# eliasandronicou/split-learning-k8s

Measured on AMD Instinct MI355X. Metric: training samples/sec (node) for split CNN, higher is better.
Workload: dtype fp32; 1 GPU; K2: split CNN (model_def.py ModelPartA+ModelPartB) both stages fused on 1xMI355X, synthetic 1x28x28 MNIST-shape batches, fp32, HIP-graph step; global_batch=4096, per_gpu_batch=4096, topology=fused-1gpu, graph=True, conv=x3, cut_handoff=client conv1 writes the x3 split input images (slk_conv1_fwd_x3); no f32 cut, client_backward=fused into the x3 dgrad (slk_conv2_dgrad_x3_c1w); no cut gradient in HBM

## Files before the change

### split-learning-k8s_amd/csrc/slk_x3.hip

```cpp
#include "slk_common.h"

#include <type_traits>

using namespace slk;

typedef _Float16 f16x8 __attribute__((ext_vector_type(8)));
typedef _Float16 f16x2 __attribute__((ext_vector_type(2)));

namespace {

constexpr int X3_SMAX = 126;
__device__ __forceinline__ int x3_exp(float amax) {
    if (!(amax > 0.f) || !__builtin_isfinite(amax)) return 0;
    int e;
    (void)frexpf(amax, &e);
    return min(14 - e, X3_SMAX);
}
__device__ __forceinline__ float x3_unscale(float v, float u1, float u2) { return (v * u1) * u2; }

__device__ __forceinline__ void x3_split8(const float* v, float sc, f16x8& h, f16x8& l) {
#pragma unroll
    for (int k = 0; k < 8; k += 2) {
        const float a = v[k] * sc, b = v[k + 1] * sc;
        const _Float16 ha = (_Float16)a, hb = (_Float16)b;
// ... 922 lines not shown
            }
        } else {
            float* gb = cut_grad + (size_t)b * A_SAMPLE + (16 * nt + n16) * A_PIX;
#pragma unroll
            for (int i = 0; i < X3D_MPW; ++i) {
                const int t = T0 + g + 4 * i, p = 16 * t + 4 * kc;
                if (t < T1 && p < A_PIX)
                    *reinterpret_cast<float4*>(gb + p) =
                        make_float4(x3_unscale(acc[i][0], us1, us2), x3_unscale(acc[i][1], us1, us2),
                                    x3_unscale(acc[i][2], us1, us2), x3_unscale(acc[i][3], us1, us2));
            }
        }
        ++q;
    }
    X3D_TS(127, 7);
    if constexpr (C1W) {
        __syncthreads();
        const float* part = reinterpret_cast<const float*>(d1s);
        if (tid < C1 * 10) {
            const int ci = tid / 10, j = tid - (tid / 10) * 10;
            const int ntc = ci >> 4, cl = ci & 15;
            const int src = ((cl >> 2) * 16 + j) * 4 + (cl & 3);
            float sum = 0.f;
            for (int gg = 0; gg < 4; ++gg) sum += part[(ntc + 2 * gg) * 256 + src];
            c1slabs[(size_t)blockIdx.x * (C1 * 10) + (j < 9 ? ci * 9 + j : C1 * 9 + ci)] = sum * ldexpf(1.f, -sw);
        }
    }
}

constexpr int X3W_THREADS = 512;
constexpr int X3W_Q = 192;
constexpr int X3W_DYP = X3W_Q * 64;
constexpr int X3W_XP = 260 * 64;
constexpr int X3W_BUF = 2 * X3W_DYP + 2 * X3W_XP;
constexpr int X3W_NKS = 128;
constexpr int X3W_XITEMS = 260 * 4;
constexpr int X3W_XR = (X3W_XITEMS + X3W_THREADS - 1) / X3W_THREADS;
constexpr int X3W_DYITEMS = 48 * 8;
static_assert(X3W_DYITEMS % 64 == 0, "whole waves of dY items");
static_assert(2 * X3W_BUF <= 163840, "LDS");

__global__ __launch_bounds__(X3W_THREADS, 1) void conv2_wgrad_x3_kernel(
    const float* __restrict__ act, const float* __restrict__ act_amax, const float* __restrict__ dpooled,
    const float* __restrict__ dp_amax, const uint8_t* __restrict__ code, float* __restrict__ slabs, int B) {
    __shared__ __attribute__((aligned(1024))) char smem[2 * X3W_BUF];
    const int tid = threadIdx.x, lane = tid & 63;
    const int wave = __builtin_amdgcn_readfirstlane(tid >> 6);
    const int h = wave & 1, kp = (wave >> 1) & 1, tg = wave >> 2;
    const int nks = (int)gridDim.x / 2;
    const int bid = blockIdx.x;
    const bool xcd = (nks & 7) == 0;
    const int cohalf = xcd ? (bid >> 3) & 1 : bid & 1;
    const int ks = xcd ? (bid >> 4) * 8 + (bid & 7) : bid >> 1;
    const int U = 3 * B;
    float* red = reinterpret_cast<float*>(smem);

    float ma = 0.f, md = 0.f;
    for (int i = tid; i < B; i += X3W_THREADS) {
        ma = fmaxf(ma, act_amax[i]);
        md = fmaxf(md, dp_amax[i]);
    }
    ma = wave_max(ma);
    md = wave_max(md);
    if (lane == 0) {
        red[wave] = ma;
        red[8 + wave] = md;
    }
    __syncthreads();
    ma = red[0];
    md = red[8];
#pragma unroll
    for (int i = 1; i < 8; ++i) {
        ma = fmaxf(ma, red[i]);
        md = fmaxf(md, red[8 + i]);
    }
    __syncthreads();
    const int sx = x3_exp(ma), sd = x3_exp(md);
    int sb_ld = 0;

    float xv[X3W_XR][8];
    auto load_x = [&](int uu) {
        const int b = uu / 3, t3 = uu - (uu / 3) * 3;
        const float* base = act + (size_t)b * A_SAMPLE + t3 * 8 * A_HW;
#pragma unroll
        for (int r = 0; r < X3W_XR; ++r) {
            const int i = min(tid + r * X3W_THREADS, X3W_XITEMS - 1);
            const int cg = i & 3, p = i >> 2;
#pragma unroll
            for (int j = 0; j < 8; ++j) xv[r][j] = base[(8 * cg + j) * A_PIX + p];
        }
    };
    auto split_x = [&](char* img) {
        const float xsc = ldexpf(1.f, sb_ld);
#pragma unroll
        for (int r = 0; r < X3W_XR; ++r) {
            const int i = min(tid + r * X3W_THREADS, X3W_XITEMS - 1);
            const int cg = i & 3, p = i >> 2;
            f16x8 hh, ll;
            x3_split8(xv[r], xsc, hh, ll);
            char* o = img + 2 * X3W_DYP + p * 64 + cg * 16;
            *reinterpret_cast<f16x8*>(o) = hh;
            *reinterpret_cast<f16x8*>(o + X3W_XP) = ll;
        }
    };
    const int ditem = min(tid, X3W_DYITEMS - 1);
    const int dg = ditem & 7, dw = ditem >> 3;
    float dv[4];
    uint32_t dcb[4];
    auto load_dy = [&](int uu) {
        const int b = uu / 3, t3 = uu - (uu / 3) * 3;
        const int w = (4 * t3 + dw / 12) * P_HW + dw % 12;
        const size_t o = (size_t)b * P_SAMPLE + (32 * cohalf + 4 * dg) * P_WIN + w;
#pragma unroll
        for (int j = 0; j < 4; ++j) {
            dv[j] = dpooled[o + j * P_WIN];
            dcb[j] = code[o + j * P_WIN];
        }
        sb_ld = max(x3_exp(act_amax[b]), sx);
    };
    float dbacc[4] = {0.f, 0.f, 0.f, 0.f};
    auto store_dy = [&](char* img, bool real) {
        const float dsc = ldexpf(1.f, sd + sx - sb_ld);
        const bool mine = real && tid < X3W_DYITEMS;
#pragma unroll
        for (int j = 0; j < 4; ++j) dbacc[j] = (mine && dcb[j] != (uint32_t)CODE_NONE) ? dbacc[j] + dv[j] : dbacc[j];
        uint32_t hv[2], lv[2];
#pragma unroll
        for (int j = 0; j < 4; j += 2) {
            const float a = dv[j] * dsc, c = dv[j + 1] * dsc;
            const _Float16 ha = (_Float16)a, hc = (_Float16)c;
            const _Float16 la = (_Float16)(a - (float)ha), lc = (_Float16)(c - (float)hc);
            hv[j / 2] = __builtin_bit_cast(uint32_t, f16x2{ha, hc});
            lv[j / 2] = __builtin_bit_cast(uint32_t, f16x2{la, lc});
        }
        const uint32_t dc = dcb[0] | (dcb[1] << 8) | (dcb[2] << 16) | (dcb[3] << 24);
        const uint32_t cA = __builtin_amdgcn_perm(0u, dc, 0x01010000u), cB = __builtin_amdgcn_perm(0u, dc, 0x03030202u);
        const int wy = dw / 12, wx = dw % 12;
        const int pf = dw & 1;
#pragma unroll
        for (int pos0 = 0; pos0 < 4; ++pos0) {
            const int pos = pos0 ^ pf;
            const uint32_t T = 0xFFu << (8 * pos);
            const uint32_t mA = __builtin_amdgcn_perm(0u, T, cA), mB = __builtin_amdgcn_perm(0u, T, cB);
            const int q = (2 * wy + (pos >> 1)) * 24 + 2 * wx + (pos & 1);
            char* o = img + q * 64 + ((((dg >> 2) ^ (q >> 3)) & 1) * 32) + 8 * (dg & 3);
            *reinterpret_cast<uint2*>(o) = make_uint2(hv[0] & mA, hv[1] & mB);
            *reinterpret_cast<uint2*>(o + X3W_DYP) = make_uint2(lv[0] & mA, lv[1] & mB);
        }
    };

    const int g4 = lane >> 4, qq = (lane >> 2) & 3, pp = lane & 3;
    int abase[3][2];
    int xbase[3][3];
#pragma unroll
    for (int j = 0; j < 3; ++j) {
        const int idx = 2 * (kp + 2 * j) + (g4 >> 1);
        const int orow = 2 * (idx / 3) + (g4 & 1), seg = idx % 3;
        const int q0 = 24 * orow + 8 * seg;
#pragma unroll
        for (int mi = 0; mi < 2; ++mi) abase[j][mi] = (q0 + qq) * 64 + ((mi ^ ((q0 >> 3) & 1)) * 32) + pp * 8;
#pragma unroll
        for (int kx = 0; kx < 3; ++kx) {
            const int x = 8 * seg + qq + kx;
            xbase[j][kx] = 2 * X3W_DYP + ((orow * A_HW + x) * 64) + h * 32 + pp * 8;
        }
    }
    typedef __fp16 hf4 __attribute__((__vector_size__(8)));
    typedef _Float16 f16x4 __attribute__((ext_vector_type(4)));
    typedef __attribute__((address_space(3))) hf4* lp4;
    auto trr = [&](const char* p) -> f16x8 {
        const f16x4 lo = __builtin_bit_cast(f16x4, __builtin_amdgcn_ds_read_tr16_b64_v4f16((lp4)p));
        const f16x4 hi = __builtin_bit_cast(f16x4, __builtin_amdgcn_ds_read_tr16_b64_v4f16((lp4)(p + 4 * 64)));
        return __builtin_shufflevector(lo, hi, 0, 1, 2, 3, 4, 5, 6, 7);
    };

    f32x4 acc[2][5];
#pragma unroll
    for (int mi = 0; mi < 2; ++mi)
#pragma unroll
        for (int t = 0; t < 5; ++t) acc[mi][t] = f32x4{0.f, 0.f, 0.f, 0.f};

    auto unit_mfma = [&](const char* img, auto TG) {
        constexpr int T0 = decltype(TG)::value ? 5 : 0, NT = decltype(TG)::value ? 4 : 5;
        constexpr int N = 3 * NT;
        f16x8 Ah[2][2], Al[2][2], Bh[3], Bl[3];
        auto rdA = [&](int j, int slot) {
#pragma unroll
            for (int mi = 0; mi < 2; ++mi) {
                Ah[slot][mi] = trr(img + abase[j][mi]);
                Al[slot][mi] = trr(img + X3W_DYP + abase[j][mi]);
            }
        };
        auto rdB = [&](int n, int slot) {
            const int j = n / NT, tap = T0 + n % NT;
            const int to = (tap / 3) * A_HW * 64;
            Bh[slot] = trr(img + xbase[j][tap % 3] + to);
            Bl[slot] = trr(img + X3W_XP + xbase[j][tap % 3] + to);
        };
        rdA(0, 0);
        rdB(0, 0);
        rdB(1, 1);
#pragma unroll
        for (int n = 0; n < N; ++n) {
            if (n + 2 < N) {
                rdB(n + 2, (n + 2) % 3);
                if ((n + 2) % NT == 0) rdA((n + 2) / NT, ((n + 2) / NT) & 1);
            }
            const int j = n / NT, t = n % NT;
#pragma unroll
            for (int mi = 0; mi < 2; ++mi)
                acc[mi][t] = mfma_x3(Ah[j & 1][mi], Al[j & 1][mi], Bh[n % 3], Bl[n % 3], acc[mi][t]);
        }
        __builtin_amdgcn_sched_group_barrier(0x100, 16, 0);
#pragma unroll
        for (int n = 0; n < N; ++n) {
            __builtin_amdgcn_sched_group_barrier(0x008, 6, 0);
            if (n + 2 < N) {
                if ((n + 2) % NT == 0) __builtin_amdgcn_sched_group_barrier(0x100, 12, 0);
                else __builtin_amdgcn_sched_group_barrier(0x100, 4, 0);
            }
        }
    };

    const int per = (U + nks - 1) / nks;
    const int u0 = min(ks * per, U), u1 = min(u0 + per, U);
    int u = u0;
    if (u < u1) {
        load_x(u);
        load_dy(u);
        split_x(smem);
        store_dy(smem, true);
        load_x(min(u + 1, u1 - 1));
        load_dy(min(u + 1, u1 - 1));
    }
    int k = 0;
#pragma unroll 1
    for (; u < u1; ++u, ++k) {
        __syncthreads();
        const int nx = u + 1, nx2 = u + 2;
        const char* img = smem + (k & 1) * X3W_BUF;
        char* nimg = smem + ((k & 1) ^ 1) * X3W_BUF;
        store_dy(nimg, nx < u1);
        split_x(nimg);
        load_x(min(nx2, u1 - 1));
        load_dy(min(nx2, u1 - 1));
        if (tg == 0) unit_mfma(img, std::integral_constant<int, 0>{});
        else unit_mfma(img, std::integral_constant<int, 1>{});
    }
    asm volatile("s_waitcnt vmcnt(0)" ::: "memory");
    __syncthreads();
    constexpr int XN = 2 * 5 * 4;
    float* xch = reinterpret_cast<float*>(smem) + (h + 2 * tg) * (XN * 64);
    if (kp == 1) {
#pragma unroll
        for (int mi = 0; mi < 2; ++mi) {
#pragma unroll
            for (int t = 0; t < 5; ++t)
#pragma unroll
                for (int r = 0; r < 4; ++r) xch[((mi * 5 + t) * 4 + r) * 64 + lane] = acc[mi][t][r];
        }
    }
    float* dbs = reinterpret_cast<float*>(smem) + 4 * XN * 64;
    if (tid < X3W_DYITEMS)
#pragma unroll
        for (int j = 0; j < 4; ++j) dbs[tid * 4 + j] = dbacc[j];
    __syncthreads();
    if (tid < 32) {
        const int g = tid >> 2, j = tid & 3;
        float sum = 0.f;
        for (int w = 0; w < 48; ++w) sum += dbs[(w * 8 + g) * 4 + j];
        slabs[(size_t)ks * (W2_N + C2) + W2_N + 32 * cohalf + tid] = sum;
    }
    if (kp == 0) {
        const float us1 = ldexpf(1.f, -sx), us2 = ldexpf(1.f, -sd);
        float* slab = slabs + (size_t)ks * (W2_N + C2);
        const int ci = 16 * h + (lane & 15);
        const int nt = tg ? 4 : 5;
#pragma unroll
        for (int mi = 0; mi < 2; ++mi) {
#pragma unroll
            for (int t = 0; t < 5; ++t)
                if (t < nt)
#pragma unroll
                    for (int r = 0; r < 4; ++r) {
                        const int co = 32 * cohalf + 16 * mi + 4 * (lane >> 4) + r;
                        slab[(co * C1 + ci) * 9 + 5 * tg + t] =
                            x3_unscale(acc[mi][t][r] + xch[((mi * 5 + t) * 4 + r) * 64 + lane], us1, us2);
                    }
        }
    }
}

constexpr int X3P_THREADS = 512;
constexpr int X3P_STEPS = 3;
constexpr int X3P_REC = X3P_STEPS * 4 * 64 * 16;
constexpr int X3P_IDXB = X3P_STEPS * 4 * 64 * 2;
constexpr int X3P_DYOFF = 2 * X3F_PLANE;
constexpr int X3P_IDXOFF = X3P_DYOFF + 2 * X3P_REC;
constexpr int X3P_BUF = (X3P_IDXOFF + X3P_IDXB + 1023) / 1024 * 1024;
constexpr int X3P_ITEMS = C2 * 12;
constexpr int X3P_SBN = (163840 - 2 * X3P_BUF) / 4;
static_assert(2 * X3P_BUF <= 163840 && X3P_ITEMS <= 2 * X3P_THREADS && X3P_ITEMS > X3P_THREADS, "x3p layout");

template <int TGI>
struct X3pTaps {
    static constexpr int NT = TGI == 0 ? 3 : 2;
    static constexpr int tap(int t) { return TGI == 0 ? t : (TGI == 1 ? 3 + t : (TGI == 2 ? 5 + t : 7 + t)); }
};

template <int TGI>
__device__ __forceinline__ void x3p_steps(const char* img, const int (&pb)[X3P_STEPS][4], const int (&sw)[3], int arec,
                                          int aidx, f32x4 (&acc)[3][4]) {
    using TT = X3pTaps<TGI>;
    constexpr int NT = TT::NT;
    typedef __fp16 hf4 __attribute__((__vector_size__(8)));
    typedef _Float16 f16x4 __attribute__((ext_vector_type(4)));
    typedef _Float16 f16x16 __attribute__((ext_vector_type(16)));
    typedef __attribute__((address_space(3))) hf4* lp4;
    auto tr = [&](const char* p) -> f16x4 { return __builtin_bit_cast(f16x4, __builtin_amdgcn_ds_read_tr16_b64_v4f16((lp4)p)); };
#pragma unroll
    for (int s = 0; s < X3P_STEPS; ++s) {
        f16x8 ah[4], al[4];
        int ix[4];
#pragma unroll
        for (int mt = 0; mt < 4; ++mt) {
            ah[mt] = *reinterpret_cast<const f16x8*>(img + X3P_DYOFF + arec + s * 4096 + mt * 256);
            al[mt] = *reinterpret_cast<const f16x8*>(img + X3P_DYOFF + X3P_REC + arec + s * 4096 + mt * 256);
            ix[mt] = *reinterpret_cast<const uint16_t*>(img + X3P_IDXOFF + aidx + s * 512 + mt * 32);
        }
#pragma unroll
        for (int t = 0; t < NT; ++t) {
            const int tap = TT::tap(t), ky = tap / 3, kx = tap % 3;
            f16x4 bh[4], bl[4];
#pragma unroll
            for (int jb = 0; jb < 4; ++jb) {
                const char* p = img + pb[s][jb] + sw[kx] + (ky * A_HW + kx) * 64;
                bh[jb] = tr(p);
                bl[jb] = tr(p + X3F_PLANE);
            }
            const f16x16 Bh = __builtin_shufflevector(__builtin_shufflevector(bh[0], bh[1], 0, 1, 2, 3, 4, 5, 6, 7),
                                                      __builtin_shufflevector(bh[2], bh[3], 0, 1, 2, 3, 4, 5, 6, 7),
                                                      0, 1, 2, 3, 4, 5, 6, 7, 8, 9, 10, 11, 12, 13, 14, 15);
            const f16x16 Bl = __builtin_shufflevector(__builtin_shufflevector(bl[0], bl[1], 0, 1, 2, 3, 4, 5, 6, 7),
                                                      __builtin_shufflevector(bl[2], bl[3], 0, 1, 2, 3, 4, 5, 6, 7),
                                                      0, 1, 2, 3, 4, 5, 6, 7, 8, 9, 10, 11, 12, 13, 14, 15);
#pragma unroll
            for (int mt = 0; mt < 4; ++mt) {
                f32x4 c = acc[t][mt];
                c = __builtin_amdgcn_smfmac_f32_16x16x64_f16(ah[mt], Bh, c, ix[mt], 0, 0);
                c = __builtin_amdgcn_smfmac_f32_16x16x64_f16(ah[mt], Bl, c, ix[mt], 0, 0);
                c = __builtin_amdgcn_smfmac_f32_16x16x64_f16(al[mt], Bh, c, ix[mt], 0, 0);
                acc[t][mt] = c;
            }
        }
    }
}

__global__ __launch_bounds__(X3P_THREADS, 1) void conv2_wgrad_x3p_kernel(
    const uint16_t* __restrict__ act16, const float* __restrict__ act_amax, const float* __restrict__ dpooled,
    const float* __restrict__ dp_amax, const uint8_t* __restrict__ code, float* __restrict__ slabs, int B) {
    __shared__ __attribute__((aligned(1024))) char smem[163840];
    int* sbt = reinterpret_cast<int*>(smem + 2 * X3P_BUF);
    const int tid = threadIdx.x, lane = tid & 63;
    const int wave = __builtin_amdgcn_readfirstlane(tid >> 6);
    const int h = wave & 1, tgi = ((wave >> 1) & 1) * 2 + (wave >> 2);
    const int ks = blockIdx.x, nks = gridDim.x;
    const int U = 3 * B;
    float* red = reinterpret_cast<float*>(smem);
    X3P_TS(0, 7);

    float ma = 0.f, md = 0.f;
    for (int i = tid; i < B; i += X3P_THREADS) {
        ma = fmaxf(ma, act_amax[i]);
        md = fmaxf(md, dp_amax[i]);
    }
    ma = wave_max(ma);
    md = wave_max(md);
    if (lane == 0) {
        red[wave] = ma;
        red[16 + wave] = md;
    }
    __syncthreads();
    ma = red[0];
    md = red[16];
#pragma unroll
    for (int i = 1; i < 8; ++i) {
        ma = fmaxf(ma, red[i]);
        md = fmaxf(md, red[16 + i]);
    }
    __syncthreads();
    const int sx = x3_exp(ma), sd = x3_exp(md);

    constexpr int NI = 2;
    const int nit = wave < 4 ? 2 : 1;
    int goff[NI], ldo[NI][2];
#pragma unroll
    for (int r = 0; r < NI; ++r) {
        const int q = r == 0 ? wave : 8 + (wave & 3);
        const int wyl = q / 3, wq = q - (q / 3) * 3;
        goff[r] = lane * P_WIN + wyl * P_HW + 4 * wq;
#pragma unroll
        for (int d = 0; d < 2; ++d) {
            const int L = 6 * (2 * wyl + d) + 2 * wq;
            const int st = L >> 4, gb = (L >> 2) & 3, jb = L & 3;
            const int rec = (st * 4 + 2 * (jb >> 1) + (gb >> 1)) * 64 + lane;
            ldo[r][d] = rec * 16 + 8 * (gb & 1);
        }
    }
    float4 dv[NI];
    uint32_t dcw[NI];
    int ld_b = 0, sb0 = 0;
    auto load_dy = [&](int uu) {
        const int b = uu / 3, t3 = uu - (uu / 3) * 3;
        const size_t o = (size_t)b * P_SAMPLE + t3 * 4 * P_HW;
#pragma unroll
        for (int r = 0; r < NI; ++r) {
            if (r < nit) {
                dv[r] = *reinterpret_cast<const float4*>(dpooled + o + goff[r]);
                dcw[r] = *reinterpret_cast<const uint32_t*>(code + o + goff[r]);
            }
        }
        ld_b = b;
    };
    float dbacc[NI] = {};
    int trk = 0;
    (void)trk;
    auto store_dy1 = [&](char* img, bool real, int r) {
        const float dsc = ldexpf(1.f, sbt[ld_b - sb0]);
        {
            {
                const float v[4] = {dv[r].x, dv[r].y, dv[r].z, dv[r].w};
#if SLK_X3D_TRACE
                if (r == 0) {
                    asm volatile("" ::"v"(v[0]), "v"(dcw[0]));
                    X3P_TS(trk, 4);
                }
#endif
                const uint32_t cw = dcw[r];
                const uint32_t ib = (cw & 1u) | ((cw >> 6) & 4u) | ((cw >> 12) & 16u) | ((cw >> 18) & 64u) | 0x88u;
#pragma unroll
                for (int j = 0; j < 4; ++j) {
                    const uint32_t c = (cw >> (8 * j)) & 0xFFu;
                    if (real && c < (uint32_t)CODE_NONE) dbacc[r] += v[j];
                }
                const uint32_t rowp = (cw >> 1) & 0x7F7F7F7Fu;
                uint32_t H[2], Lw[2];
#pragma unroll
                for (int jp = 0; jp < 2; ++jp) {
                    const float a = v[2 * jp] * dsc, bb = v[2 * jp + 1] * dsc;
                    const _Float16 ha = (_Float16)a, hb = (_Float16)bb;
                    const _Float16 la = (_Float16)(a - (float)ha), lb = (_Float16)(bb - (float)hb);
                    H[jp] = __builtin_bit_cast(uint32_t, f16x2{ha, hb});
                    Lw[jp] = __builtin_bit_cast(uint32_t, f16x2{la, lb});
                }
#pragma unroll
                for (int d = 0; d < 2; ++d) {
                    const uint32_t z = (d ? (rowp & ~(rowp >> 1)) : ~(rowp | (rowp >> 1))) & 0x01010101u;
                    const uint32_t m8 = z * 0xFFu;
                    const uint32_t mA = __builtin_amdgcn_perm(0u, m8, 0x01010000u), mB = __builtin_amdgcn_perm(0u, m8, 0x03030202u);
                    char* ph = img + X3P_DYOFF + ldo[r][d];
                    *reinterpret_cast<uint2*>(ph) = make_uint2(H[0] & mA, H[1] & mB);
                    *reinterpret_cast<uint2*>(ph + X3P_REC) = make_uint2(Lw[0] & mA, Lw[1] & mB);
                    img[X3P_IDXOFF + ((ldo[r][d] >> 4) << 1) + ((ldo[r][d] >> 3) & 1)] = (char)ib;
                }
            }
        }
    };
    auto store_dy = [&](char* img, bool real) {
#pragma unroll
        for (int r = 0; r < NI; ++r)
            if (r < nit) store_dy1(img, real, r);
        X3P_TS(trk, 5);
    };

    const int gbl = lane >> 4, qq = (lane >> 2) & 3, pp = lane & 3;
    int pb[X3P_STEPS][4], sw[3];
#pragma unroll
    for (int s = 0; s < X3P_STEPS; ++s)
#pragma unroll
        for (int jb = 0; jb < 4; ++jb) {
            const int L = 16 * s + 4 * gbl + jb, y = L / 6, xb = L - (L / 6) * 6;
            pb[s][jb] = (y * A_HW + 4 * xb + qq) * 64 + pp * 8;
        }
#pragma unroll
    for (int kx = 0; kx < 3; ++kx) sw[kx] = (h ^ (((kx + qq) >> 1) & 1)) * 32;
    const int arec = ((lane >> 4) * 64 + (lane & 15)) * 16, aidx = ((lane >> 4) * 64 + (lane & 15)) * 2;

    f32x4 acc[3][4];
#pragma unroll
    for (int t = 0; t < 3; ++t)
#pragma unroll
        for (int mt = 0; mt < 4; ++mt) acc[t][mt] = f32x4{0.f, 0.f, 0.f, 0.f};

    const int per = (U + nks - 1) / nks;
    const int u0 = min(ks * per, U), u1 = min(u0 + per, U);
    sb0 = u0 / 3;
    const int nsb = u1 > u0 ? (u1 - 1) / 3 - sb0 + 1 : 0;
    for (int j = tid; j < nsb; j += X3P_THREADS) sbt[j] = sd + sx - max(x3_exp(act_amax[sb0 + j]), sx);
    __syncthreads();
    int u = u0;
    if (u < u1) {
        x3_issue_unit_img(act16, u, wave, lane, lds_u32(smem));
        load_dy(u);
        store_dy(smem, true);
        load_dy(min(u + 1, u1 - 1));
    }
    int k = 0;
#pragma unroll 1
    for (; u < u1; ++u, ++k) {
        X3P_TS(k, 6);
        if (nit == 2) asm volatile("s_waitcnt vmcnt(4)" ::: "memory");
        else asm volatile("s_waitcnt vmcnt(2)" ::: "memory");
        __syncthreads();
        X3P_TS(k, 0);
        trk = k;
        const int nx = u + 1, nx2 = u + 2;
        const char* img = smem + (k & 1) * X3P_BUF;
        char* nimg = smem + ((k & 1) ^ 1) * X3P_BUF;
        const bool dfirst = wave >= 4;
        if (dfirst) store_dy(nimg, nx < u1);
        x3_issue_unit_img(act16, min(nx, u1 - 1), wave, lane, lds_u32(nimg));
        if (dfirst) load_dy(min(nx2, u1 - 1));
        X3P_TS(k, 1);
        if (tgi == 0) x3p_steps<0>(img, pb, sw, arec, aidx, acc);
        else if (tgi == 1) x3p_steps<1>(img, pb, sw, arec, aidx, acc);
        else if (tgi == 2) x3p_steps<2>(img, pb, sw, arec, aidx, acc);
        else x3p_steps<3>(img, pb, sw, arec, aidx, acc);
        X3P_TS(k, 2);
        if (!dfirst) {
            store_dy(nimg, nx < u1);
            load_dy(min(nx2, u1 - 1));
        }
        X3P_TS(k, 3);
    }
    X3P_TS(127, 7);
    asm volatile("s_waitcnt vmcnt(0)" ::: "memory");
    __syncthreads();
    float* dbs = reinterpret_cast<float*>(smem);
#pragma unroll
    for (int r = 0; r < NI; ++r)
        if (r < nit) dbs[(r == 0 ? wave : 8 + (wave & 3)) * 64 + lane] = dbacc[r];
    __syncthreads();
    float* slab = slabs + (size_t)ks * (W2_N + C2);
    if (tid < C2) {
        float sum = 0.f;
        for (int q = 0; q < 12; ++q) sum += dbs[q * 64 + tid];
        slab[W2_N + tid] = sum;
    }
    const float us1 = ldexpf(1.f, -sx), us2 = ldexpf(1.f, -sd);
    const int ci = 16 * h + (lane & 15);
    auto write_slab = [&](auto TG) {
        using TT = X3pTaps<decltype(TG)::value>;
#pragma unroll
        for (int t = 0; t < TT::NT; ++t)
#pragma unroll
            for (int mt = 0; mt < 4; ++mt)
#pragma unroll
                for (int r = 0; r < 4; ++r) {
                    const int co = 16 * mt + 4 * (lane >> 4) + r;
                    slab[(co * C1 + ci) * 9 + TT::tap(t)] = x3_unscale(acc[t][mt][r], us1, us2);
                }
    };
    if (tgi == 0) write_slab(std::integral_constant<int, 0>{});
    else if (tgi == 1) write_slab(std::integral_constant<int, 1>{});
    else if (tgi == 2) write_slab(std::integral_constant<int, 2>{});
    else write_slab(std::integral_constant<int, 3>{});
}

constexpr int C1X_T = 256;
constexpr int C1X_G = A_PIX / 4;
static_assert(RB_SAMPLE == 4 * C1X_G, "bit map layout");
template <bool BITS, bool ACT>
__global__ __launch_bounds__(C1X_T) void conv1_fwd_x3_kernel(const float* __restrict__ x, const float* __restrict__ W1,
                                                             const float* __restrict__ b1, float* __restrict__ act,
                                                             float* __restrict__ act_amax, uint16_t* __restrict__ act16,
                                                             uint32_t* __restrict__ relu_bits) {
    __shared__ float xs[IN_HW * IN_HW];
    __shared__ float red[8];
    __shared__ float ws[C1 * 10];
    const int b = blockIdx.x;
    const int tid = threadIdx.x;
    const float* xb = x + (size_t)b * IN_HW * IN_HW;
    for (int i = tid; i < IN_HW * IN_HW / 4; i += C1X_T)
        reinterpret_cast<float4*>(xs)[i] = reinterpret_cast<const float4*>(xb)[i];
    for (int i = tid; i < C1 * 9; i += C1X_T) ws[(i / 9) * 10 + i % 9] = W1[i];
    if (tid < C1) ws[tid * 10 + 9] = b1[tid];
    __syncthreads();
    const float am = conv1_cut_bound(xs, W1, b1, red);
    if (tid == 0) act_amax[b] = am;
    const float sc = ldexpf(1.f, x3_exp(am));
    const int c8 = tid & 3;
    float wr[8][10];
#pragma unroll
    for (int j = 0; j < 8; ++j)
#pragma unroll
        for (int k = 0; k < 10; ++k) wr[j][k] = ws[(8 * c8 + j) * 10 + k];
    char* img = reinterpret_cast<char*>(act16) + (size_t)b * X3S_SAMPLE;
    float* actb = ACT ? act + (size_t)b * A_SAMPLE : nullptr;
#pragma unroll 2
    for (int i = tid; i < A_PIX * 4; i += C1X_T) {
        const int p = i >> 2;
        const int y = p / A_HW, xx = p - (p / A_HW) * A_HW;
        float xw[9];
#pragma unroll
        for (int k = 0; k < 9; ++k) xw[k] = xs[(y + k / 3) * IN_HW + xx + k % 3];
        float v[8];
#pragma unroll
        for (int j = 0; j < 8; ++j) {
            float sum = 0.f;
#pragma unroll
            for (int k = 0; k < 9; ++k) sum = fmaf(xw[k], wr[j][k], sum);
            sum += wr[j][9];
            v[j] = sum > 0.f ? sum : 0.f;
        }
        if constexpr (ACT) {
#pragma unroll
            for (int j = 0; j < 8; ++j) actb[(8 * c8 + j) * A_PIX + p] = v[j];
        }
        if constexpr (BITS) {
            const int u = p & 3;
            uint32_t w = 0u;
#pragma unroll
            for (int j = 0; j < 8; ++j) w |= min(__float_as_uint(v[j]), 1u) << (4 * j);
            w <<= u;
            w |= (uint32_t)__builtin_amdgcn_ds_swizzle((int)w, (4 << 10) | 0x1F);
            w |= (uint32_t)__builtin_amdgcn_ds_swizzle((int)w, (8 << 10) | 0x1F);
            if (u == 0) relu_bits[(size_t)b * RB_SAMPLE + c8 * C1X_G + (p >> 2)] = w;
        }
        f16x8 hh, ll;
        x3_split8(v, sc, hh, ll);
        char* o = img + p * 64 + (c8 ^ (xx & 2)) * 16;
        *reinterpret_cast<f16x8*>(o) = hh;
        *reinterpret_cast<f16x8*>(o + X3S_PLANE) = ll;
    }
}

__global__ __launch_bounds__(C1X_T) void cut_unpack_x3_kernel(const float* __restrict__ vals,
                                                              const uint32_t* __restrict__ mask,
                                                              const int* __restrict__ ranks,
                                                              const float* __restrict__ amax,
                                                              uint16_t* __restrict__ act16,
                                                              const uint64_t* __restrict__ parts = nullptr,
                                                              int part_b = 0) {
    constexpr int NW = A_SAMPLE / 32;
    __shared__ uint32_t sm[NW];
    __shared__ int sr[NW];
    const int b = blockIdx.x, tid = threadIdx.x;
    int lb = b;
    if (parts != nullptr) {
        const int part = b / part_b;
        lb = b - part * part_b;
        vals = reinterpret_cast<const float*>(parts[3 * part]);
        mask = reinterpret_cast<const uint32_t*>(parts[3 * part + 1]);
        ranks = reinterpret_cast<const int*>(parts[3 * part + 2]);
    }
    for (int i = tid; i < NW; i += C1X_T) {
        sm[i] = mask[(size_t)lb * NW + i];
        sr[i] = ranks[(size_t)lb * NW + i];
    }
    __syncthreads();
    const float sc = ldexpf(1.f, x3_exp(amax[b]));
    const int c8 = tid & 3;
    char* img = reinterpret_cast<char*>(act16) + (size_t)b * X3S_SAMPLE;
#pragma unroll 1
    for (int i = tid; i < A_PIX * 4; i += C1X_T) {
        const int p = i >> 2, xx = p - (p / A_HW) * A_HW;
        float v[8];
#pragma unroll
        for (int j = 0; j < 8; ++j) {
            const int e = (8 * c8 + j) * A_PIX + p, w = e >> 5, bit = e & 31;
            const uint32_t m = sm[w];
            v[j] = 0.f;
            if ((m >> bit) & 1u) v[j] = vals[(size_t)sr[w] + __popc(m & ((1u << bit) - 1u))];
        }
        f16x8 hh, ll;
        x3_split8_img(v, sc, hh, ll);
        char* o = img + p * 64 + (c8 ^ (xx & 2)) * 16;
        *reinterpret_cast<f16x8*>(o) = hh;
        *reinterpret_cast<f16x8*>(o + X3S_PLANE) = ll;
    }
}

extern "C" int slk_cut_unpack_x3(const float* vals, const uint32_t* mask, const int* ranks, const float* act_amax,
                                 int B, uint16_t* act16, void* stream) {
    SLK_CHECK_ARG(B >= 0 && (int64_t)B * A_SAMPLE <= 2147483647LL);
    if (B == 0) return 0;
    SLK_CHECK_ARG(vals && mask && ranks && act_amax && act16);
    hipLaunchKernelGGL(cut_unpack_x3_kernel, dim3(B), dim3(C1X_T), 0, slk_stream(stream), vals, mask, ranks, act_amax,
                       act16, nullptr, 0);
    return slk_launch_status();
}

extern "C" int slk_cut_unpack_x3_parts(const uint64_t* parts, int part_b, const float* act_amax, int B, uint16_t* act16,
                                       void* stream) {
    SLK_CHECK_ARG(B >= 0 && part_b > 0 && B % part_b == 0 && (int64_t)part_b * A_SAMPLE <= 2147483647LL);
    if (B == 0) return 0;
    SLK_CHECK_ARG(parts && act_amax && act16);
    hipLaunchKernelGGL(cut_unpack_x3_kernel, dim3(B), dim3(C1X_T), 0, slk_stream(stream), nullptr, nullptr, nullptr,
                       act_amax, act16, parts, part_b);
    return slk_launch_status();
}

__global__ __launch_bounds__(256) void mfma_probe_kernel(float* __restrict__ out, int iters) {
    const int tid = threadIdx.x;
    f16x8 a, b;
#pragma unroll
    for (int j = 0; j < 8; ++j) {
        a[j] = (_Float16)((float)((tid * 13 + j * 7 + blockIdx.x) % 97) / 97.f - 0.5f);
        b[j] = (_Float16)((float)((tid * 29 + j * 11) % 89) / 89.f - 0.5f);
    }
    f32x4 c0 = {0.f, 0.f, 0.f, 0.f}, c1 = c0, c2 = c0, c3 = c0, c4 = c0, c5 = c0;
    for (int i = 0; i < iters; ++i)
        asm volatile(
            "v_mfma_f32_16x16x32_f16 %0, %6, %7, %0\n\t"
            "v_mfma_f32_16x16x32_f16 %1, %6, %7, %1\n\t"
            "v_mfma_f32_16x16x32_f16 %2, %6, %7, %2\n\t"
            "v_mfma_f32_16x16x32_f16 %3, %6, %7, %3\n\t"
            "v_mfma_f32_16x16x32_f16 %4, %6, %7, %4\n\t"
            "v_mfma_f32_16x16x32_f16 %5, %6, %7, %5"
            : "+v"(c0), "+v"(c1), "+v"(c2), "+v"(c3), "+v"(c4), "+v"(c5)
            : "v"(a), "v"(b));
    asm volatile("s_nop 7\n\ts_nop 7" ::: "memory");
    const f32x4 t4 = ((c0 + c1) + (c2 + c3)) + (c4 + c5);
    out[blockIdx.x * 256 + tid] = (t4[0] + t4[1]) + (t4[2] + t4[3]);
}

extern "C" int slk_mfma_probe_blocks() { return 2 * X3F_GRID; }

extern "C" int slk_mfma_probe(float* out, int iters, void* stream) {
    SLK_CHECK_ARG(out && iters > 0);
    hipLaunchKernelGGL(mfma_probe_kernel, dim3(2 * X3F_GRID), dim3(256), 0, slk_stream(stream), out, iters);
    return slk_launch_status();
}

extern "C" int slk_row_amax(const float* x, int rows, int n, float* amax, void* stream) {
    SLK_CHECK_ARG(rows >= 0 && n > 0 && (rows == 0 || (x && amax)));
    if (rows == 0) return 0;
    hipLaunchKernelGGL(row_amax_kernel, dim3(rows), dim3(256), 0, slk_stream(stream), x, n, amax);
    return slk_launch_status();
}

extern "C" int slk_conv2_fwd_pool_x3s(const float* act, const float* act_amax, const float* W2, const float* b2,
                                      float* pooled, uint8_t* code, uint16_t* act16, int B, void* stream) {
    SLK_CHECK_ARG(B >= 0 && act && act_amax && W2 && b2 && pooled && code && act16);
    if (B == 0) return 0;
    const int U = 3 * B;
    hipLaunchKernelGGL(conv2_fwd_pool_x3_kernel<false>, dim3(U < X3F_GRID ? U : X3F_GRID), dim3(X3F_THREADS), 0,
                       slk_stream(stream), act, act_amax, W2, b2, pooled, code, B, act16);
    return slk_launch_status();
}
extern "C" int slk_conv2_fwd_pool_x3sa(const float* act, float* act_amax, const float* W2, const float* b2,
                                       float* pooled, uint8_t* code, uint16_t* act16, int B, void* stream) {
    SLK_CHECK_ARG(B >= 0 && act && act_amax && W2 && b2 && pooled && code && act16);
    if (B == 0) return 0;
    SLK_CHECK_ARG((reinterpret_cast<size_t>(act) & 15) == 0);
    const int G = B < X3F_GRID ? B : X3F_GRID;
    hipLaunchKernelGGL((conv2_fwd_pool_x3_kernel<false, true>), dim3(G), dim3(X3F_THREADS), 0, slk_stream(stream),
                       act, nullptr, W2, b2, pooled, code, B, act16, act_amax);
    return slk_launch_status();
}
extern "C" int64_t slk_conv2_act16_bytes(int B) { return B > 0 ? (int64_t)B * X3S_SAMPLE : 0; }

extern "C" int slk_conv2_fwd_pool_x3(const float* act, const float* act_amax, const float* W2, const float* b2,
                                     float* pooled, uint8_t* code, int B, void* stream) {
    SLK_CHECK_ARG(B >= 0 && act && act_amax && W2 && b2 && pooled && code);
    if (B == 0) return 0;
    const int U = 3 * B;
    hipLaunchKernelGGL(conv2_fwd_pool_x3_kernel<false>, dim3(U < X3F_GRID ? U : X3F_GRID), dim3(X3F_THREADS), 0,
                       slk_stream(stream), act, act_amax, W2, b2, pooled, code, B, nullptr);
    return slk_launch_status();
}

extern "C" int slk_conv2_fwd_pool_x3i(const uint16_t* act16, const float* act_amax, const float* W2, const float* b2,
                                      float* pooled, uint8_t* code, int B, void* stream) {
    SLK_CHECK_ARG(B >= 0 && act16 && act_amax && W2 && b2 && pooled && code);
    if (B == 0) return 0;
    const int U = 3 * B;
    hipLaunchKernelGGL(conv2_fwd_pool_x3_kernel<true>, dim3(U < X3F_GRID ? U : X3F_GRID), dim3(X3F_THREADS), 0,
                       slk_stream(stream), nullptr, act_amax, W2, b2, pooled, code, B, const_cast<uint16_t*>(act16));
    return slk_launch_status();
}

extern "C" int slk_conv2_fwd_pool_x3p(const uint16_t* act16, const float* act_amax, const float* W2, const float* b2,
                                      float* pooled, int B, void* stream) {
    SLK_CHECK_ARG(B >= 0);
    if (B == 0) return 0;
    SLK_CHECK_ARG(act16 && act_amax && W2 && b2 && pooled);
    const int U = 3 * B;
    hipLaunchKernelGGL((conv2_fwd_pool_x3_kernel<true, false, false>), dim3(U < X3F_GRID ? U : X3F_GRID),
                       dim3(X3F_THREADS), 0, slk_stream(stream), nullptr, act_amax, W2, b2, pooled, nullptr, B,
                       const_cast<uint16_t*>(act16));
    return slk_launch_status();
}

extern "C" int slk_conv1_fwd_x3(const float* x, const float* W1, const float* b1, float* act, float* act_amax,
                                uint16_t* act16, uint32_t* relu_bits, int B, void* stream) {
    SLK_CHECK_ARG(B >= 0 && (B == 0 || (x && W1 && b1 && act_amax && act16)));
    if (B == 0) return 0;
    const dim3 g(B), t(C1X_T);
    if (relu_bits && act)
        hipLaunchKernelGGL((conv1_fwd_x3_kernel<true, true>), g, t, 0, slk_stream(stream), x, W1, b1, act, act_amax, act16, relu_bits);
    else if (relu_bits)
        hipLaunchKernelGGL((conv1_fwd_x3_kernel<true, false>), g, t, 0, slk_stream(stream), x, W1, b1, act, act_amax, act16, relu_bits);
    else if (act)
        hipLaunchKernelGGL((conv1_fwd_x3_kernel<false, true>), g, t, 0, slk_stream(stream), x, W1, b1, act, act_amax, act16, relu_bits);
    else
        hipLaunchKernelGGL((conv1_fwd_x3_kernel<false, false>), g, t, 0, slk_stream(stream), x, W1, b1, act, act_amax, act16, relu_bits);
    return slk_launch_status();
}
extern "C" int64_t slk_relu_bits_bytes(int B) { return B > 0 ? (int64_t)B * RB_SAMPLE * 4 : 0; }

extern "C" int slk_conv2_dgrad_x3(const float* dpooled, const float* dp_amax, const uint8_t* code, const float* W2,
                                  float* cut_grad, int B, void* stream) {
    SLK_CHECK_ARG(B >= 0 && dpooled && dp_amax && code && W2 && cut_grad);
    if (B == 0) return 0;
    const int P = 3 * B;
    hipLaunchKernelGGL(conv2_dgrad_x3_kernel<false>, dim3(P < X3D_GRID ? P : X3D_GRID), dim3(X3D_THREADS), 0,
                       slk_stream(stream), dpooled, dp_amax, code, W2, cut_grad, B, nullptr, nullptr, nullptr);
    return slk_launch_status();
}

extern "C" int slk_conv2_dgrad_x3_pack(const float* dpooled, const float* dp_amax, const uint8_t* code, const float* W2,
                                       const uint32_t* mask, const int* ranks, float* vals, int B, void* stream) {
    SLK_CHECK_ARG(B >= 0 && (int64_t)B * A_SAMPLE <= 2147483647LL);
    if (B == 0) return 0;
    SLK_CHECK_ARG(dpooled && dp_amax && code && W2 && mask && ranks && vals);
    const int P = 3 * B;
    hipLaunchKernelGGL(conv2_dgrad_x3_kernel<false>, dim3(P < X3D_GRID ? P : X3D_GRID), dim3(X3D_THREADS), 0,
                       slk_stream(stream), dpooled, dp_amax, code, W2, nullptr, B, nullptr, nullptr, nullptr, mask, ranks,
                       vals);
    return slk_launch_status();
}

extern "C" int slk_conv2_dgrad_x3_pack_parts(const float* dpooled, const float* dp_amax, const uint8_t* code,
                                             const float* W2, const uint64_t* parts, int part_b, int B, void* stream) {
    SLK_CHECK_ARG(B >= 0 && part_b > 0 && B % part_b == 0 && (int64_t)part_b * A_SAMPLE <= 2147483647LL);
    if (B == 0) return 0;
    SLK_CHECK_ARG(dpooled && dp_amax && code && W2 && parts);
    const int P = 3 * B;
    hipLaunchKernelGGL(conv2_dgrad_x3_kernel<false>, dim3(P < X3D_GRID ? P : X3D_GRID), dim3(X3D_THREADS), 0,
                       slk_stream(stream), dpooled, dp_amax, code, W2, nullptr, B, nullptr, nullptr, nullptr, nullptr,
                       nullptr, nullptr, parts, part_b);
    return slk_launch_status();
}

extern "C" int slk_conv2_dgrad_x3_c1w_nslab(int B) { return B <= 0 ? 0 : (3 * B < X3D_GRID ? 3 * B : X3D_GRID); }

extern "C" int slk_conv2_dgrad_x3_c1w(const float* dpooled, const float* dp_amax, const uint8_t* code, const float* W2,
                                      const float* x, const uint32_t* relu_bits, float* client_slabs, int B,
                                      void* stream) {
    SLK_CHECK_ARG(B >= 0 && (B == 0 || (dpooled && dp_amax && code && W2 && x && relu_bits && client_slabs)));
    if (B == 0) return 0;
    const int P = 3 * B;
    hipLaunchKernelGGL(conv2_dgrad_x3_kernel<true>, dim3(P < X3D_GRID ? P : X3D_GRID), dim3(X3D_THREADS), 0,
                       slk_stream(stream), dpooled, dp_amax, code, W2, nullptr, B, x, relu_bits, client_slabs);
    return slk_launch_status();
}

constexpr int X3_WGRAD_NSLAB = 256;
extern "C" int slk_conv2_wgrad_x3_nslab(int B) { return B <= 0 ? 0 : (6 * B < X3_WGRAD_NSLAB ? 6 * B : X3_WGRAD_NSLAB); }

extern "C" int slk_conv2_wgrad_x3(const float* act, const float* act_amax, const float* dpooled, const float* dp_amax,
                                  const uint8_t* code, float* slabs, int B, void* stream) {
// ... 36 lines not shown
```

Before: 5.125 million samples/s.

## Remap x3p wgrad K-blocks to row/column layout with swizzled image staging

Changes the mapping of the conv2 weight-gradient K dimension so each staging item writes one contiguous 16-byte dy record and one 16-bit index word, instead of two 8-byte halves and two index bytes. B-operand addresses are recomputed from a single per-kx base plus a row and step offset, which drops the per-step pb/sw register tables. The image is staged through a new issue routine whose source offsets are XOR-swizzled to match the new LDS slot layout. The intent is fewer LDS stores, fewer bank conflicts and lower register pressure, at the cost of more intricate indexing guarded by constexpr bijectivity checks.

```diff
diff --git a/split-learning-k8s_amd/csrc/slk_x3.hip b/split-learning-k8s_amd/csrc/slk_x3.hip
--- a/split-learning-k8s_amd/csrc/slk_x3.hip
+++ b/split-learning-k8s_amd/csrc/slk_x3.hip
@@ -1248,22 +1248,81 @@
 constexpr int X3P_SBN = (163840 - 2 * X3P_BUF) / 4;
 static_assert(2 * X3P_BUF <= 163840 && X3P_ITEMS <= 2 * X3P_THREADS && X3P_ITEMS > X3P_THREADS, "x3p layout");
 
+constexpr int x3p_row(int gb, int jb) { return 4 * (gb >> 1) + jb; }
+constexpr int x3p_cb(int s, int gb) { return 2 * s + (gb & 1); }
+constexpr int x3p_item_ga(int wyl) { return 2 * (wyl & 1) + (wyl >> 1); }
+constexpr bool x3p_kmap_bijective() {
+    unsigned long long seen = 0;
+    for (int s = 0; s < X3P_STEPS; ++s)
+        for (int gb = 0; gb < 4; ++gb)
+            for (int jb = 0; jb < 4; ++jb) {
+                const int r = x3p_row(gb, jb), cb = x3p_cb(s, gb);
+                if (r < 0 || r >= 8 || cb < 0 || cb >= 6 || ((seen >> (6 * r + cb)) & 1)) return false;
+                seen |= 1ull << (6 * r + cb);
+            }
+    return seen == (1ull << 48) - 1;
+}
+constexpr bool x3p_items_cover_records() {
+    unsigned seen = 0;
+    for (int wyl = 0; wyl < 4; ++wyl)
+        for (int wq = 0; wq < 3; ++wq) {
+            const int s = wq, ga = x3p_item_ga(wyl);
+            if ((seen >> (4 * s + ga)) & 1) return false;
+            seen |= 1u << (4 * s + ga);
+            for (int i = 0; i < 8; ++i) {
+                const int gb = 2 * (ga & 1) + (i >> 2), jb = 2 * (ga >> 1) + ((i >> 1) & 1);
+                const int r = x3p_row(gb, jb), cb = x3p_cb(s, gb);
+                if ((r >> 1) != wyl || (cb >> 1) != wq || (cb & 1) != (i >> 2) || (r & 1) != ((i >> 1) & 1)) return false;
+            }
+        }
+    return seen == (1u << 12) - 1;
+}
+static_assert(x3p_kmap_bijective(), "(s, gb, jb) <-> (row, column block) over the unit's 48 blocks");
+static_assert(x3p_items_cover_records(), "every record and index word is written by exactly one staging item");
+
+
+__device__ __host__ constexpr int x3p_slot(int h, int x) { return h ^ ((x >> 1) & 1) ^ ((x >> 2) & 1); }
+__device__ __host__ constexpr uint32_t x3p_img_src(int T) {
+    return (uint32_t)(T ^ (((((T >> 6) % A_HW) >> 2) & 1) << 5));
+}
+__device__ __forceinline__ void x3p_issue_unit_img(const uint16_t* act16, int uu, int wave, int lane, uint32_t lds,
+                                                   const uint32_t (&dvo)[5]) {
+    const int b = uu / 3, t3 = uu - (uu / 3) * 3;
+    const char* srch = reinterpret_cast<const char*>(act16) + (size_t)b * X3S_SAMPLE + t3 * X3S_UNIT_OFF;
+    constexpr int PP = X3F_PLANE / 1024 + 1;
+#pragma unroll
+    for (int r = 0; r < 5; ++r) {
+        const int piece = wave + 8 * r;
+        if (piece < 2 * PP) {
+            const int pl = piece >= PP ? 1 : 0, pp = piece - PP * pl;
+            if (pp < PP - 1 || lane < 16) glds16_so(srch + pl * X3S_PLANE, dvo[r], lds + pl * X3F_PLANE + pp * 1024);
+        }
+    }
+}
+
 template <int TGI>
 struct X3pTaps {
     static constexpr int NT = TGI == 0 ? 3 : 2;
     static constexpr int tap(int t) { return TGI == 0 ? t : (TGI == 1 ? 3 + t : (TGI == 2 ? 5 + t : 7 + t)); }
 };
 
+typedef _Float16 x3p_f16x4 __attribute__((ext_vector_type(4)));
+typedef _Float16 x3p_f16x16 __attribute__((ext_vector_type(16)));
+__device__ __forceinline__ x3p_f16x4 x3p_tr(const char* p) {
+    typedef __fp16 hf4 __attribute__((__vector_size__(8)));
+    typedef __attribute__((address_space(3))) hf4* lp4;
+    return __builtin_bit_cast(x3p_f16x4, __builtin_amdgcn_ds_read_tr16_b64_v4f16((lp4)p));
+}
+__device__ __forceinline__ x3p_f16x16 x3p_cat4(x3p_f16x4 a, x3p_f16x4 b, x3p_f16x4 c, x3p_f16x4 d) {
+    return __builtin_shufflevector(__builtin_shufflevector(a, b, 0, 1, 2, 3, 4, 5, 6, 7),
+                                   __builtin_shufflevector(c, d, 0, 1, 2, 3, 4, 5, 6, 7), 0, 1, 2, 3, 4, 5, 6, 7, 8, 9,
+                                   10, 11, 12, 13, 14, 15);
+}
+
 template <int TGI>
-__device__ __forceinline__ void x3p_steps(const char* img, const int (&pb)[X3P_STEPS][4], const int (&sw)[3], int arec,
-                                          int aidx, f32x4 (&acc)[3][4]) {
+__device__ __forceinline__ void x3p_steps(const char* img, const int (&pk)[3], int arec, int aidx, f32x4 (&acc)[12]) {
     using TT = X3pTaps<TGI>;
     constexpr int NT = TT::NT;
-    typedef __fp16 hf4 __attribute__((__vector_size__(8)));
-    typedef _Float16 f16x4 __attribute__((ext_vector_type(4)));
-    typedef _Float16 f16x16 __attribute__((ext_vector_type(16)));
-    typedef __attribute__((address_space(3))) hf4* lp4;
-    auto tr = [&](const char* p) -> f16x4 { return __builtin_bit_cast(f16x4, __builtin_amdgcn_ds_read_tr16_b64_v4f16((lp4)p)); };
 #pragma unroll
     for (int s = 0; s < X3P_STEPS; ++s) {
         f16x8 ah[4], al[4];
@@ -1272,31 +1331,27 @@
         for (int mt = 0; mt < 4; ++mt) {
             ah[mt] = *reinterpret_cast<const f16x8*>(img + X3P_DYOFF + arec + s * 4096 + mt * 256);
             al[mt] = *reinterpret_cast<const f16x8*>(img + X3P_DYOFF + X3P_REC + arec + s * 4096 + mt * 256);
-            ix[mt] = *reinterpret_cast<const uint16_t*>(img + X3P_IDXOFF + aidx + s * 512 + mt * 32);
+            ix[mt] = *reinterpret_cast<const uint16_t*>(img + X3P_IDXOFF + aidx + (s * 4 + mt) * 128);
         }
 #pragma unroll
         for (int t = 0; t < NT; ++t) {
             const int tap = TT::tap(t), ky = tap / 3, kx = tap % 3;
-            f16x4 bh[4], bl[4];
+            x3p_f16x4 bh[4], bl[4];
 #pragma unroll
             for (int jb = 0; jb < 4; ++jb) {
-                const char* p = img + pb[s][jb] + sw[kx] + (ky * A_HW + kx) * 64;
-                bh[jb] = tr(p);
-                bl[jb] = tr(p + X3F_PLANE);
-            }
-            const f16x16 Bh = __builtin_shufflevector(__builtin_shufflevector(bh[0], bh[1], 0, 1, 2, 3, 4, 5, 6, 7),
-                                                      __builtin_shufflevector(bh[2], bh[3], 0, 1, 2, 3, 4, 5, 6, 7),
-                                                      0, 1, 2, 3, 4, 5, 6, 7, 8, 9, 10, 11, 12, 13, 14, 15);
-            const f16x16 Bl = __builtin_shufflevector(__builtin_shufflevector(bl[0], bl[1], 0, 1, 2, 3, 4, 5, 6, 7),
-                                                      __builtin_shufflevector(bl[2], bl[3], 0, 1, 2, 3, 4, 5, 6, 7),
-                                                      0, 1, 2, 3, 4, 5, 6, 7, 8, 9, 10, 11, 12, 13, 14, 15);
+                const char* p = img + pk[kx] + ((jb + ky) * A_HW + 8 * s) * 64;
+                bh[jb] = x3p_tr(p);
+                bl[jb] = x3p_tr(p + X3F_PLANE);
+            }
+            const x3p_f16x16 Bh = x3p_cat4(bh[0], bh[1], bh[2], bh[3]);
+            const x3p_f16x16 Bl = x3p_cat4(bl[0], bl[1], bl[2], bl[3]);
 #pragma unroll
             for (int mt = 0; mt < 4; ++mt) {
-                f32x4 c = acc[t][mt];
+                f32x4 c = acc[t * 4 + mt];
                 c = __builtin_amdgcn_smfmac_f32_16x16x64_f16(ah[mt], Bh, c, ix[mt], 0, 0);
                 c = __builtin_amdgcn_smfmac_f32_16x16x64_f16(ah[mt], Bl, c, ix[mt], 0, 0);
                 c = __builtin_amdgcn_smfmac_f32_16x16x64_f16(al[mt], Bh, c, ix[mt], 0, 0);
-                acc[t][mt] = c;
+                acc[t * 4 + mt] = c;
             }
         }
     }
@@ -1339,19 +1394,15 @@
 
     constexpr int NI = 2;
     const int nit = wave < 4 ? 2 : 1;
-    int goff[NI], ldo[NI][2];
+    int goff[NI], ldo[NI], ldi[NI];
 #pragma unroll
     for (int r = 0; r < NI; ++r) {
         const int q = r == 0 ? wave : 8 + (wave & 3);
         const int wyl = q / 3, wq = q - (q / 3) * 3;
         goff[r] = lane * P_WIN + wyl * P_HW + 4 * wq;
-#pragma unroll
-        for (int d = 0; d < 2; ++d) {
-            const int L = 6 * (2 * wyl + d) + 2 * wq;
-            const int st = L >> 4, gb = (L >> 2) & 3, jb = L & 3;
-            const int rec = (st * 4 + 2 * (jb >> 1) + (gb >> 1)) * 64 + lane;
-            ldo[r][d] = rec * 16 + 8 * (gb & 1);
-        }
+        const int ga = x3p_item_ga(wyl);
+        ldo[r] = ((wq * 4 + ga) * 64 + lane) * 16;
+        ldi[r] = (((wq * 4 + (lane >> 4)) * 4 + ga) * 16 + (lane & 15)) * 2;
     }
     float4 dv[NI];
     uint32_t dcw[NI];
@@ -1384,6 +1435,7 @@
 #endif
                 const uint32_t cw = dcw[r];
                 const uint32_t ib = (cw & 1u) | ((cw >> 6) & 4u) | ((cw >> 12) & 16u) | ((cw >> 18) & 64u) | 0x88u;
+                const uint32_t iw = ((ib & 0xFu) | ((ib & 0xF0u) << 4)) * 0x11u;
 #pragma unroll
                 for (int j = 0; j < 4; ++j) {
                     const uint32_t c = (cw >> (8 * j)) & 0xFFu;
@@ -1399,16 +1451,18 @@
                     H[jp] = __builtin_bit_cast(uint32_t, f16x2{ha, hb});
                     Lw[jp] = __builtin_bit_cast(uint32_t, f16x2{la, lb});
                 }
+                uint32_t mA[2], mB[2];
 #pragma unroll
                 for (int d = 0; d < 2; ++d) {
                     const uint32_t z = (d ? (rowp & ~(rowp >> 1)) : ~(rowp | (rowp >> 1))) & 0x01010101u;
                     const uint32_t m8 = z * 0xFFu;
-                    const uint32_t mA = __builtin_amdgcn_perm(0u, m8, 0x01010000u), mB = __builtin_amdgcn_perm(0u, m8, 0x03030202u);
-                    char* ph = img + X3P_DYOFF + ldo[r][d];
-                    *reinterpret_cast<uint2*>(ph) = make_uint2(H[0] & mA, H[1] & mB);
-                    *reinterpret_cast<uint2*>(ph + X3P_REC) = make_uint2(Lw[0] & mA, Lw[1] & mB);
-                    img[X3P_IDXOFF + ((ldo[r][d] >> 4) << 1) + ((ldo[r][d] >> 3) & 1)] = (char)ib;
+                    mA[d] = __builtin_amdgcn_perm(0u, m8, 0x01010000u);
+                    mB[d] = __builtin_amdgcn_perm(0u, m8, 0x03030202u);
                 }
+                char* ph = img + X3P_DYOFF + ldo[r];
+                *reinterpret_cast<uint4*>(ph) = make_uint4(H[0] & mA[0], H[0] & mA[1], H[1] & mB[0], H[1] & mB[1]);
+                *reinterpret_cast<uint4*>(ph + X3P_REC) = make_uint4(Lw[0] & mA[0], Lw[0] & mA[1], Lw[1] & mB[0], Lw[1] & mB[1]);
+                *reinterpret_cast<uint16_t*>(img + X3P_IDXOFF + ldi[r]) = (uint16_t)iw;
             }
         }
     };
@@ -1420,23 +1474,23 @@
     };
 
     const int gbl = lane >> 4, qq = (lane >> 2) & 3, pp = lane & 3;
-    int pb[X3P_STEPS][4], sw[3];
-#pragma unroll
-    for (int s = 0; s < X3P_STEPS; ++s)
-#pragma unroll
-        for (int jb = 0; jb < 4; ++jb) {
-            const int L = 16 * s + 4 * gbl + jb, y = L / 6, xb = L - (L / 6) * 6;
-            pb[s][jb] = (y * A_HW + 4 * xb + qq) * 64 + pp * 8;
-        }
-#pragma unroll
-    for (int kx = 0; kx < 3; ++kx) sw[kx] = (h ^ (((kx + qq) >> 1) & 1)) * 32;
-    const int arec = ((lane >> 4) * 64 + (lane & 15)) * 16, aidx = ((lane >> 4) * 64 + (lane & 15)) * 2;
-
-    f32x4 acc[3][4];
-#pragma unroll
-    for (int t = 0; t < 3; ++t)
-#pragma unroll
-        for (int mt = 0; mt < 4; ++mt) acc[t][mt] = f32x4{0.f, 0.f, 0.f, 0.f};
+    int pk[3];
+#pragma unroll
+    for (int kx = 0; kx < 3; ++kx) {
+        const int x = 4 * (gbl & 1) + qq + kx;
+        pk[kx] = (x3p_row(gbl, 0) * A_HW + x) * 64 + x3p_slot(h, x) * 32 + pp * 8;
+    }
+    const int arec = ((lane >> 4) * 64 + (lane & 15)) * 16, aidx = ((lane >> 4) * 16 + (lane & 15)) * 2;
+    uint32_t dvo[5];
+#pragma unroll
+    for (int r = 0; r < 5; ++r) {
+        const int piece = wave + 8 * r, pl17 = piece >= 17 ? 1 : 0;
+        dvo[r] = x3p_img_src((piece - 17 * pl17) * 1024 + lane * 16);
+    }
+
+    f32x4 acc[12];
+#pragma unroll
+    for (int t = 0; t < 12; ++t) acc[t] = f32x4{0.f, 0.f, 0.f, 0.f};
 
     const int per = (U + nks - 1) / nks;
     const int u0 = min(ks * per, U), u1 = min(u0 + per, U);
@@ -1446,7 +1500,7 @@
     __syncthreads();
     int u = u0;
     if (u < u1) {
-        x3_issue_unit_img(act16, u, wave, lane, lds_u32(smem));
+        x3p_issue_unit_img(act16, u, wave, lane, lds_u32(smem), dvo);
         load_dy(u);
         store_dy(smem, true);
         load_dy(min(u + 1, u1 - 1));
@@ -1465,13 +1519,13 @@
         char* nimg = smem + ((k & 1) ^ 1) * X3P_BUF;
         const bool dfirst = wave >= 4;
         if (dfirst) store_dy(nimg, nx < u1);
-        x3_issue_unit_img(act16, min(nx, u1 - 1), wave, lane, lds_u32(nimg));
+        x3p_issue_unit_img(act16, min(nx, u1 - 1), wave, lane, lds_u32(nimg), dvo);
         if (dfirst) load_dy(min(nx2, u1 - 1));
         X3P_TS(k, 1);
-        if (tgi == 0) x3p_steps<0>(img, pb, sw, arec, aidx, acc);
-        else if (tgi == 1) x3p_steps<1>(img, pb, sw, arec, aidx, acc);
-        else if (tgi == 2) x3p_steps<2>(img, pb, sw, arec, aidx, acc);
-        else x3p_steps<3>(img, pb, sw, arec, aidx, acc);
+        if (tgi == 0) x3p_steps<0>(img, pk, arec, aidx, acc);
+        else if (tgi == 1) x3p_steps<1>(img, pk, arec, aidx, acc);
+        else if (tgi == 2) x3p_steps<2>(img, pk, arec, aidx, acc);
+        else x3p_steps<3>(img, pk, arec, aidx, acc);
         X3P_TS(k, 2);
         if (!dfirst) {
             store_dy(nimg, nx < u1);
@@ -1504,7 +1558,7 @@
 #pragma unroll
                 for (int r = 0; r < 4; ++r) {
                     const int co = 16 * mt + 4 * (lane >> 4) + r;
-                    slab[(co * C1 + ci) * 9 + TT::tap(t)] = x3_unscale(acc[t][mt][r], us1, us2);
+                    slab[(co * C1 + ci) * 9 + TT::tap(t)] = x3_unscale(acc[t * 4 + mt][r], us1, us2);
                 }
     };
     if (tgi == 0) write_slab(std::integral_constant<int, 0>{});
```

Measured after the change: 5.119 million samples/s. No clear change (-0.1%).
